# aelefebv/nellie

Measured on AMD Instinct MI355X. Metric: Mvoxel/s multiscale Frangi (5 sigma) + Label, float32, frame resident in HBM, higher is better.
Workload: dtype f32; 1 GPU; synthetic 1024x1024x1024 float32 volume (N(100,5) noise + Gaussian tube segments, seed 2345), 0.1 um isotropic, 5-scale Frangi + Label, full hot path per step, frame resident in HBM; voxels=1073741824, labels=265, one_pass_scales=5, fast_div_proven=2, hessian_tile_rows=16

## Files before the change

nellie_amd/csrc/hessian.inc:

```
struct VessP {
    float gamma_sq, alpha_sq, beta_sq;
    int use_thr;
    float thr;
    float max_abs, max_finite;
    int have_prev;
    int cnt_lo, cnt_hi;
    int first;
    float fsq_min;
    int m_inf;
    unsigned int *nan_flag;
    int all_ones;
    float fsq_lo, fsq_hi;
    int qcap;
    int zchunk;
    i64 idx_lo, idx_hi;
};

#define HM_TRACE_C 0.30f
#define HM_ENT 28
struct __attribute__((packed, aligned(4))) QEnt4 { float a, b, c, d; };
struct __attribute__((packed, aligned(4))) QEnt3 { float a, b, c; };
__device__ __forceinline__ void qent_store(float4 *region, unsigned int slot, float h0, float h1, float h2, float h3, float h4, float h5, unsigned int idx) {
    char *e = reinterpret_cast<char *>(region) + (size_t)__umul24(slot, (unsigned int)HM_ENT);
    *reinterpret_cast<QEnt4 *>(e) = QEnt4{h0, h1, h2, h3};
// ... 328 lines not shown
        mabs = wave_max_f(mabs); mfrob = wave_max_f(mfrob); anyinf = wave_or_i(anyinf);
        if ((tid & 63) == 0) { s_red[w] = mabs; s_red[16 + w] = mfrob; s_red[32 + w] = anyinf ? 1.0f : 0.0f; }
        __syncthreads();
        if (tid == 0) {
            float a = 0.0f, b = 0.0f, c = 0.0f;
            for (int k = 0; k < NT / 64; ++k) { a = fmaxf(a, s_red[k]); b = fmaxf(b, s_red[16 + k]); c = fmaxf(c, s_red[32 + k]); }
            if (a > 0.0f && __float_as_uint(a) > __hip_atomic_load(&res[0], __ATOMIC_RELAXED, __HIP_MEMORY_SCOPE_AGENT)) atomicMax(&res[0], __float_as_uint(a));
            if (b > 0.0f && __float_as_uint(b) > __hip_atomic_load(&res[1], __ATOMIC_RELAXED, __HIP_MEMORY_SCOPE_AGENT)) atomicMax(&res[1], __float_as_uint(b));
            if (c > 0.0f) atomicOr(&res[2], 1u);
        }
    }
    if (MODE != 0) {
        __syncthreads();
        if (lane == 0) {
            vq.count[region] = qn;
            if (MODE == 2 && qn > (unsigned int)vp.qcap) atomicOr(&res[3], 1u);
        }
        unsigned int *s_cnt = (unsigned int *)s_red;
        if (lane == 0) s_cnt[w] = cnt;
        __syncthreads();
        if (tid == 0) {
            unsigned long long t = 0;
            for (int k = 0; k < NT / 64; ++k) t += s_cnt[k];
            if (t) atomicAdd(mask_count, t);
        }
    }
}

template <bool RESOLVE>
__global__ void __launch_bounds__(256)
vesselness_queue_kernel(const float4 *__restrict__ ent, const unsigned int *__restrict__ count, unsigned int nregions,
                        float *__restrict__ vmax, i64 base, VessP vp, unsigned long long *cmask64,
                        const unsigned long long *pmask64, int wpr, int ny, int nx, i64 zbase,
                        unsigned long long *__restrict__ mask_count, const float *__restrict__ dev_params) {
    if (dev_params) { vp.gamma_sq = dev_params[2]; vp.fsq_min = dev_params[3]; vp.m_inf = __float_as_int(dev_params[4]); }
    unsigned int passed = 0;
    bool st_pending = false;
    i64 st_at = 0;
    float st_val = 0.0f;
    const unsigned int rstep = gridDim.x * 4u;
    unsigned int r = blockIdx.x * 4u + (threadIdx.x >> 6);
    unsigned int n_next = r < nregions ? count[r] : 0u;
    for (; r < nregions; r += rstep) {
    unsigned int n = n_next;
    n_next = (r + rstep < nregions) ? count[r + rstep] : 0u;
    if (RESOLVE && n > (unsigned int)vp.qcap) n = (unsigned int)vp.qcap;
    const float4 *e = ent + (size_t)r * (size_t)vp.qcap * 2;
    unsigned int i = threadIdx.x & 63u;
    float4 a = make_float4(0.f, 0.f, 0.f, 0.f), b = a;
    if (i < n) qent_load(e, i, a, b);
    asm volatile("" :: "v"(a.x), "v"(b.x));
    for (; i < n; i += 64u) {
        if (st_pending) { vmax[st_at] = st_val; st_pending = false; }
        const float4 a0 = a, b0 = b;
        if (i + 64u < n) qent_load(e, i + 64u, a, b);
        const float h[6] = {a0.x, a0.y, a0.z, a0.w, b0.x, b0.y};
        if (vp.all_ones) {
            if ((h[0] != h[0]) | (h[1] != h[1]) | (h[2] != h[2]) | (h[3] != h[3]) | (h[4] != h[4]) | (h[5] != h[5])) *vp.nan_flag = 1u;
        }
        unsigned int idx = __float_as_uint(b0.z);
        const bool undecided = RESOLVE && (idx & HM_UNDECIDED);
        idx &= ~HM_UNDECIDED;
        const i64 c = base + idx;
        const float cur = vp.first ? 0.0f : vmax[c];
        if (undecided) {
            const float fsq = frob_sq_of(h);
            if (!((fsq >= vp.fsq_min) && (fsq < __int_as_float(0x7f800000) || vp.m_inf))) continue;
            if ((i64)idx >= vp.idx_lo && (i64)idx < vp.idx_hi) ++passed;
            const i64 plane = (i64)ny * nx;
            const i64 zl = idx / plane;
            const int rem = (int)(idx - zl * plane);
            const int yy = rem / nx, xx = rem - yy * nx;
            const i64 word = ((zbase + zl) * ny + yy) * wpr + (xx >> 6);
            const unsigned long long bit = 1ull << (xx & 63);
            if (vp.have_prev && !(pmask64[word] & bit)) continue;
            atomicOr(&cmask64[word], bit);
            const float tr = h[0] + h[3] + h[5];
            if (!HM_TRACE_OK(tr, fsq)) continue;
        }
        float l1, l2, l3;
        eig3_sorted_abs(h, l1, l2, l3);
        const float val = frangi3(l1, l2, l3, vp.alpha_sq, vp.beta_sq, vp.gamma_sq);
        if (val > cur) { st_pending = true; st_at = c; st_val = val; }
    }
    }
    if (st_pending) vmax[st_at] = st_val;
    if (RESOLVE) {
        unsigned long long t = wave_sum_u64((unsigned long long)passed);
// ... 294 lines not shown
```

nellie_amd/csrc/label_runs.inc:

```

struct RunRec { int row; unsigned int x; };
struct RunN { const unsigned int *p; i64 h; i64 cap; };
__device__ __forceinline__ i64 run_n(const RunN &r) { const i64 n = r.p ? (i64)*r.p : r.h; return n > r.cap ? 0 : n; }

__device__ __forceinline__ unsigned long long rl_word(const unsigned long long *__restrict__ bits, i64 row, int w, int wpr,
                                                      int nx, bool invert) {
    unsigned long long v = bits[row * wpr + w];
    if (invert) v = ~v;
    const int rem = nx - w * 64;
    if (rem < 64) v &= (rem <= 0) ? 0ull : ((1ull << rem) - 1ull);
    return v;
}

__global__ void __launch_bounds__(256)
rl_threshold_pack_kernel(const float *__restrict__ f, const unsigned long long *__restrict__ support, unsigned long long *__restrict__ bits,
                         int has_thr, float thr_host, int nx, i64 nrows, int wpr, const float *__restrict__ thr_dev = nullptr) {
    const float thr = thr_dev ? *thr_dev : thr_host;
    const i64 wstride = ((i64)gridDim.x * blockDim.x) >> 6;
    const int lane = threadIdx.x & 63;
    const bool row_words = support && wpr <= 64;
    const i64 first = ((i64)blockIdx.x * blockDim.x + threadIdx.x) >> 6;
    unsigned long long mine_next = (row_words && first < nrows && lane < wpr) ? support[first * wpr + lane] : 0ull;
    unsigned long long st_res = 0ull;
    i64 st_row = -1;
// ... 430 lines not shown
    __syncthreads();
    const i64 base = chunk * RL_CHUNK;
    for (int k = threadIdx.x; k < RL_CHUNK; k += 256) {
        const i64 i = base + k;
        if (i >= nruns) break;
        const int root = parent[i];
        const int len = (int)(runs[i].x >> 16) - (int)(runs[i].x & 0xffffu);
        unsigned int h = ((unsigned int)root * 2654435761u) >> 24;
        bool done = false;
        for (int probe = 0; probe < 8 && !done; ++probe) {
            const int old = atomicCAS(&keys[h], -1, root);
            if (old == -1 || old == root) { atomicAdd(&vals[h], len); done = true; }
            else h = (h + 1) & (RL_HT - 1);
        }
        if (!done) atomicAdd(&area[root], len);
    }
    __syncthreads();
    for (int k = threadIdx.x; k < RL_HT; k += 256)
        if (keys[k] >= 0 && vals[k]) atomicAdd(&area[keys[k]], vals[k]);
  }
}

__global__ void __launch_bounds__(256)
rl_keep_kernel(const RunRec *__restrict__ runs, const int *__restrict__ parent, const int *__restrict__ area, int min_area,
               unsigned long long *__restrict__ bits, RunN rn, int wpr) {
    const i64 nruns = run_n(rn);
    for (i64 i = (i64)blockIdx.x * blockDim.x + threadIdx.x; i < nruns; i += (i64)gridDim.x * blockDim.x) {
        if (area[parent[i]] < min_area) continue;
        const RunRec r = runs[i];
        rl_set_bits(bits, r.row, wpr, (int)(r.x & 0xffffu), (int)(r.x >> 16));
    }
}

__global__ void __launch_bounds__(256)
majority_bits_kernel(const unsigned long long *__restrict__ in, unsigned long long *__restrict__ out, VolGeom v, int wpr, i64 z_lo, i64 z_hi) {
    const unsigned int ny = (unsigned int)v.ny, uw = (unsigned int)wpr;
    const unsigned int nw = (unsigned int)(z_hi - z_lo) * ny * uw;
    const unsigned int t0 = blockIdx.x * blockDim.x + threadIdx.x;
    if (t0 >= nw) return;
    const unsigned int w = t0 % uw, row0 = t0 / uw;
    const int y = (int)(row0 % ny), z = (int)(row0 / ny) + (int)z_lo;
    const i64 t = ((i64)z * ny + y) * wpr + w;
    const bool last = (w == uw - 1u);
    const unsigned long long top = 1ull << (((int)v.nx - 1) & 63);
    const unsigned long long valid = (top << 1) - 1ull;
    unsigned long long c0 = 0, c1 = 0, c2 = 0, c3 = 0, c4 = 0;
    auto add = [&](unsigned long long b) {
        unsigned long long t0_ = c0 & b; c0 ^= b; b = t0_;
        t0_ = c1 & b; c1 ^= b; b = t0_;
        t0_ = c2 & b; c2 ^= b; b = t0_;
        t0_ = c3 & b; c3 ^= b; b = t0_;
        c4 ^= b;
    };
    unsigned long long cw[9];
    i64 rws[9];
    unsigned long long any = 0ull;
#pragma unroll
    for (int dz = -1; dz <= 1; ++dz) {
        int zz = z + dz;
        const i64 gg = v.gz0 + zz;
        if (gg < 0 || gg >= v.gnz) zz = z;
#pragma unroll
        for (int dy = -1; dy <= 1; ++dy) {
            int yy = y + dy;
            yy = yy < 0 ? 0 : (yy >= (int)ny ? (int)ny - 1 : yy);
            const int k = (dz + 1) * 3 + (dy + 1);
            rws[k] = ((i64)zz * ny + yy) * wpr;
            cw[k] = in[rws[k] + w];
            any |= cw[k];
        }
    }
    if (any == 0ull) { out[t] = 0ull; return; }
#pragma unroll
    for (int k = 0; k < 9; ++k) {
        const unsigned long long cur = cw[k];
        const unsigned long long prev = (w > 0u) ? in[rws[k] + w - 1] : 0ull;
        const unsigned long long left = (cur << 1) | ((w > 0u) ? (prev >> 63) : (cur & 1ull));
        const unsigned long long next = last ? 0ull : in[rws[k] + w + 1];
        const unsigned long long right = (cur >> 1) | (last ? (cur & top) : (next << 63));
        add(left); add(cur); add(right);
    }
    unsigned long long res = c4 | (c3 & c2 & c1);
    if (last) res &= valid;
    out[t] = res;
}

__global__ void __launch_bounds__(256)
rl_paint_kernel(const unsigned long long *__restrict__ bits, const unsigned int *__restrict__ row_off, const int *__restrict__ parent,
                const int *__restrict__ newid, int *__restrict__ out, i64 row0, i64 row1, int wpr, int nx) {
    const i64 wstride = ((i64)gridDim.x * blockDim.x) >> 6;
    const int lane = threadIdx.x & 63;
    for (i64 row = row0 + (((i64)blockIdx.x * blockDim.x + threadIdx.x) >> 6); row < row1; row += wstride) {
        const unsigned int seen0 = row_off[row], nr = row_off[row + 1] - seen0;
        unsigned int seen = seen0;
        int *orow = out + (row - row0) * nx;
        const bool vec = ((nx & 3) == 0) && ((reinterpret_cast<size_t>(orow) & 15) == 0);
        if (nr == 0u && vec) {
            for (int q = lane; q < nx / 4; q += 64) reinterpret_cast<int4 *>(orow)[q] = make_int4(0, 0, 0, 0);
            continue;
        }
        const int lab_mine = ((unsigned int)lane < nr) ? newid[parent[seen0 + lane]] : 0;
        if (vec) {
            for (int q = lane; q < nx / 4; q += 64) reinterpret_cast<int4 *>(orow)[q] = make_int4(0, 0, 0, 0);
            asm volatile("s_waitcnt vmcnt(0)" ::: "memory");
            unsigned long long carry = 0;
            int prev_w = -2;
            for (int wb = 0; wb < wpr; wb += 64) {
                const unsigned long long mine = (wb + lane < wpr) ? rl_word(bits, row, wb + lane, wpr, nx, false) : 0ull;
                unsigned long long todo = __ballot(mine != 0ull);
                while (todo) {
                    const int wl = __builtin_ctzll(todo);
                    todo &= todo - 1;
                    const int w = wb + wl;
                    const unsigned long long v = __shfl(mine, wl, 64);
                    if (w != prev_w + 1) carry = 0ull;
                    const unsigned long long starts = v & ~((v << 1) | carry);
                    const int x = w * 64 + lane;
// ... 174 lines not shown
```

nellie_amd/csrc/nellie_hip.hip:

```cpp
#include "nl_host.h"

struct RcclApi {
    void *handle = nullptr;
    decltype(&ncclGetUniqueId) GetUniqueId = nullptr;
    decltype(&ncclCommInitRank) CommInitRank = nullptr;
    decltype(&ncclCommDestroy) CommDestroy = nullptr;
    decltype(&ncclGetErrorString) GetErrorString = nullptr;
    decltype(&ncclGroupStart) GroupStart = nullptr;
    decltype(&ncclGroupEnd) GroupEnd = nullptr;
    decltype(&ncclSend) Send = nullptr;
    decltype(&ncclRecv) Recv = nullptr;
    decltype(&ncclAllReduce) AllReduce = nullptr;
    decltype(&ncclBroadcast) Broadcast = nullptr;
    decltype(&ncclAllGather) AllGather = nullptr;
    bool ok = false;
};
static RcclApi &rccl_real() {
    static RcclApi api;
    if (!api.handle) {
        std::string rp;
        if (const char *e = getenv("ROCM_PATH")) rp = std::string(e) + "/lib/librccl.so.1";
        const char *names[] = {rp.c_str(), "/opt/rocm/lib/librccl.so.1", "/opt/rocm/lib/librccl.so", "librccl.so.1", "librccl.so"};
        for (const char *n : names) { if (!*n) continue; api.handle = dlopen(n, RTLD_NOW | RTLD_GLOBAL); if (api.handle) break; }
        if (api.handle) {
// ... 65 lines not shown
    return rccl_real().Broadcast(src, dst, count, dt, root, comm, st);
}
CommApi &rccl() { static CommApi api; return api; }

#include "sampling.inc"
#include "hessian.inc"
#include "hessian_pair.inc"
#include "hv_launch.h"
#include "filter2d.inc"
#include "thresholds.inc"
#include "chain.inc"
#include "percentile.inc"

static bool chain_unfused_sampling() {
    static int v = -1;
    if (v < 0) { const char *e = getenv("NELLIE_CHAIN_UNFUSED_SAMPLING"); v = (e && e[0] == '1') ? 1 : 0; }
    return v == 1;
}
static i64 sample_grid_cap() {
    static i64 v = 0;
    if (!v) { const char *e = getenv("NELLIE_SAMPLE_GRID"); v = (e && atoll(e) > 0) ? atoll(e) : 256; }
    return v;
}

bool gyx_tiled() {
    static int on = -1;
    if (on < 0) { const char *e = getenv("NELLIE_GYX_TILE"); on = (e && !atoi(e)) ? 0 : 1; }
    return on != 0;
}
static unsigned resolve_grid(unsigned blocks) {
    static long cap = -1;
    if (cap < 0) { const char *e = getenv("NELLIE_RESOLVE_GRID"); cap = e ? atol(e) : 8192; }
    return (cap > 0 && (unsigned)cap < blocks) ? (unsigned)cap : blocks;
}
static int hm_ty() {
    static int v = -1;
    if (v < 0) { const char *e = getenv("NELLIE_HM_TY"); v = (e && atoi(e) == 16) ? 16 : 8; }
    return v;
}
static int hv_rs_env() {
    static int v = -1;
    if (v < 0) { const char *e = getenv("NELLIE_HV_RS"); v = e ? atoi(e) : 8; if (v != 0 && v != 8 && !(NL_HV_VARIANTS && v == 16)) v = 8; }
    return v;
}
static int hv_rs(const nl_ctx *c) { return ((i64)(HM_ZCHUNK + 4) * c->ny * c->nx * 4 < ((i64)1 << 32)) ? hv_rs_env() : 0; }
static HessP hessp(const nl_ctx *c);
static HessDv<1> hessdv_fast(const nl_ctx *c) { return hessdv_fast(hessp(c)); }
static HessDv<0> hessdv_exact(const nl_ctx *c) { return hessdv_exact(hessp(c)); }
static int hv_fastv(const nl_ctx *c) { return c->fast_div2 ? 2 : (c->fast_div ? 1 : 0); }
static int hv_np(const nl_ctx *c) {
#if NL_HV_VARIANTS
    const char *e = getenv("NELLIE_HV_NP");
    return (e && atoi(e) == 2 && hv_rs(c) == 8 && hv_fastv(c) == 2) ? 2 : 1;
#else
    (void)c;
    return 1;
#endif
}
#define HD_SR 4
#define HD_COLS 60
static bool hv_dpp(const nl_ctx *c) {
    const char *e = getenv("NELLIE_HV_DPP");
    return hv_rs(c) != 0 && e && atoi(e) == 1;
}
static int hd_zchunk(const nl_ctx *c, i64 nz, i64 strips) {
    static int forced = -1;
// ... 1099 lines not shown
    NL_HIP(hipStreamSynchronize(st));
    *mask_count = (int64_t)(*h_cnt + c->spec_count);
    return NL_OK;
}

static bool resolve_on_side() {
    static int overlap = -1;
    if (overlap < 0) { const char *e = getenv("NELLIE_RESOLVE_OVERLAP"); overlap = (e && atoi(e)) ? 1 : 0; }
    return overlap != 0;
}
static int resolve_enqueue(nl_ctx *c, VessP vp, unsigned long long *d_cnt, const float *dev_params, char *err, size_t errlen, bool force_side = false) {
    const i64 plane = c->ny * c->nx, z0 = c->spec_z0, z1 = c->spec_z1;
    const bool side = force_side || resolve_on_side();
    hipStream_t st = side ? c->side : c->stream;
    if (side) {
        NL_HIP(hipEventRecord(c->ev_main, c->stream));
        NL_HIP(hipStreamWaitEvent(c->side, c->ev_main, 0));
    }
    vp.qcap = c->spec_qcap;
    vp.idx_lo = (c->own_lo - z0) * plane; vp.idx_hi = (c->own_hi - z0) * plane;
    {
        ProfScope ps(c, "vesselness_resolve", st);
        const int wpr = (int)((c->nx + 63) / 64);
        const i64 slot_words = c->nzl * c->ny * wpr;
        const int k_scale = c->mask_slots_used++;
        vp.have_prev = k_scale > 0;
        unsigned long long *cm = (unsigned long long *)c->m[0] + (i64)(k_scale & 1) * slot_words;
        const unsigned long long *pm = (unsigned long long *)c->m[0] + (i64)((k_scale + 1) & 1) * slot_words;
        if (vp.first && !vmax_is_zero(c, z0, z1))
            NL_HIP(hipMemsetAsync(c->f[c->i_vmax] + z0 * plane, 0, (size_t)(z1 - z0) * plane * 4, st));
        c->vmax_zero_hi = 0;
        vesselness_queue_kernel<true><<<resolve_grid((c->spec_nregions + 3) / 4), 256, 0, st>>>(
            (const float4 *)c->d_vq, c->d_vq_count, c->spec_nregions, c->f[c->i_vmax], z0 * plane, vp, cm, pm, wpr, (int)c->ny, (int)c->nx, z0, d_cnt,
            dev_params);
        NL_CHECK_LAUNCH();
    }
    if (side) {
        NL_HIP(hipEventRecord(c->ev_side, c->side));
        c->side_pending = 1;
    }
    c->spec_valid = 0;
    return NL_OK;
}

static bool resolve_defer_ok(const nl_ctx *c) {
    const char *e = getenv("NELLIE_RESOLVE_DEFER");
    const int on = e ? atoi(e) : 1;
    if (on == 2) return !c->comm && !resolve_on_side();
    return on && !c->comm && !c->ahead_pending && !resolve_on_side() && c->n >= ((i64)1 << 26);
}
static int resolve_deferred_launch(nl_ctx *c, bool on_side, char *err, size_t errlen) {
    if (!c->def_resolve) return NL_OK;
    c->def_resolve = 0;
    NL_JOIN_SIDE(c);
    VessP vp;
    static_assert(sizeof(VessP) <= sizeof(((nl_ctx *)nullptr)->def_vp), "nl_ctx::def_vp holds a VessP");
    memcpy(&vp, c->def_vp, sizeof(VessP));
    return resolve_enqueue(c, vp, c->def_cnt, c->def_params, err, errlen, on_side);
}

extern "C" int nl_vesselness_resolve(nl_ctx *c, float gamma_sq, float alpha_sq, float beta_sq, int use_thr, float thr,
                                     int *hit, int64_t *mask_count, char *err, size_t errlen) {
    NL_ENTER(c);
    if (!hit) return nl_fail(err, errlen, NL_EINVAL, "hit is NULL");
    *hit = 0;
    if (!c->spec_valid) return NL_OK;
    VessP vp = make_vessp(c, gamma_sq, alpha_sq, beta_sq, use_thr, thr);
// ... 272 lines not shown
    } else {
        ProfScope ps(c, "vesselness");
        const int ntx = (int)((c->nx + HM_TX - 1) / HM_TX);
        const int wpr = (int)((c->nx + 63) / 64);
        const i64 slot_words = c->nzl * c->ny * wpr;
        const int k_scale = c->mask_slots_used++;
        vp.have_prev = k_scale > 0;
        unsigned long long *cm = (unsigned long long *)c->m[0] + (i64)(k_scale & 1) * slot_words;
        const unsigned long long *pm = (unsigned long long *)c->m[0] + (i64)((k_scale + 1) & 1) * slot_words;
        const i64 plane = c->ny * c->nx;
        const i64 planes_per_launch = (i64)c->vq_chunks * HM_ZCHUNK;
        const VQueue vq{(float4 *)c->d_vq, c->d_vq_count};
        if (vp.first && !vmax_is_zero(c, z0, z1))
            NL_HIP(hipMemsetAsync(c->f[c->i_vmax] + z0 * plane, 0, (size_t)(z1 - z0) * plane * 4, c->stream));
        c->vmax_zero_hi = 0;
        const int rs = hv_rs(c);
        const int ty = rs ? 2 * rs : hm_ty();
        const int nty = (int)((c->ny + ty - 1) / ty);
        if (rs) vp.qcap = 2 * hv_np(c) * HM_REGION;
#define NL_LAUNCH_VESS(TYV, FASTV, HR)                                                                                    \
        hessian_g_kernel<1, TYV, FASTV><<<nblocks, HGCfg<TYV>::NT, HGCfg<TYV>::lds_bytes(), c->stream>>>(                 \
            gauss_cur(c), cm, pm, wpr, geom(c), HR, vp, vq, (int)za, (int)zb, ntx, nty, nullptr, d_cnt)
        for (i64 za = z0; za < z1; za += planes_per_launch) {
            const i64 zb = za + planes_per_launch < z1 ? za + planes_per_launch : z1;
            const int nzc = (int)((zb - za + HM_ZCHUNK - 1) / HM_ZCHUNK);
            const unsigned nblocks = (unsigned)(ntx * nty * nzc);
            if (rs) NL_HIP(nl_hv_launch(HvLaunch{1, rs, hv_np(c), hv_fastv(c), nblocks, c->stream, gauss_cur(c), cm, pm, wpr, geom(c), hessp(c), vp, vq, (int)za, (int)zb,
                                                 ntx, nty, nullptr, d_cnt, nullptr}));
            else if (ty == 8) { if (c->fast_div) NL_LAUNCH_VESS(8, true, hessdv_fast(c)); else NL_LAUNCH_VESS(8, false, hessdv_exact(c)); }
            else { if (c->fast_div) NL_LAUNCH_VESS(16, true, hessdv_fast(c)); else NL_LAUNCH_VESS(16, false, hessdv_exact(c)); }
            NL_CHECK_LAUNCH();
            const unsigned nregions = nblocks * (unsigned)(rs ? rs / hv_np(c) : ty);
            vesselness_queue_kernel<false><<<resolve_grid((nregions + 3) / 4), 256, 0, c->stream>>>(vq.ent, vq.count, nregions, c->f[c->i_vmax], za * plane, vp,
                                                                                      nullptr, nullptr, wpr, (int)c->ny, (int)c->nx, za, nullptr, nullptr);
            NL_CHECK_LAUNCH();
        }
#undef NL_LAUNCH_VESS
        NL_CHECK_LAUNCH();
    }
    if (mask_count) {
        NL_HIP(hipMemcpyAsync(c->h_small, d_cnt, 8, hipMemcpyDeviceToHost, c->stream));
        NL_HIP(hipStreamSynchronize(c->stream));
        *mask_count = (int64_t)(*(unsigned long long *)c->h_small);
    }
    return NL_OK;
}

extern "C" int nl_set_ndim(nl_ctx *c, int ndim, char *err, size_t errlen) {
    NL_ENTER(c);
    if (ndim != 2 && ndim != 3) return nl_fail(err, errlen, NL_EINVAL, "ndim must be 2 or 3");
    if (ndim == 2 && (c->nzl != 1 || c->gnz != 1)) return nl_fail(err, errlen, NL_EINVAL, "a 2-D context has exactly one plane");
    c->two_d = ndim == 2;
    c->fsq_cache_valid = 0;
    return NL_OK;
}

extern "C" int nl_log2d_step(nl_ctx *c, const double *wy2, const double *wy0, const double *wx2, const double *wx0, int r,
                             float s2, int first, int use_mask, char *err, size_t errlen) {
    NL_ENTER(c);
    if (!c->two_d) return nl_fail(err, errlen, NL_ESTATE, "nl_log2d_step on a 3-D context");
    if (!wy2 || !wy0 || !wx2 || !wx0) return nl_fail(err, errlen, NL_EINVAL, "weights are NULL");
    NL_JOIN_SIDE(c);
    for (int k = 0; k < 4; ++k)
        if (!c->d_2d[k]) NL_HIP(hipMalloc((void **)&c->d_2d[k], (size_t)c->n * 4));
    GaussW gy2, gy0, gx2, gx0;
    int rc;
    if ((rc = fill_gw(gy2, wy2, r, err, errlen)) || (rc = fill_gw(gy0, wy0, r, err, errlen)) ||
// ... 696 lines not shown
    NL_HIP(zero_small(d_n, 4, c->stream));
    {
        ProfScope ps(c, "sample");
        flat_gather_pos_kernel<<<(unsigned)((count + 255) / 256), 256, 0, c->stream>>>(src, -c->gz0 * plane, offset + k0 * step, step, count, stage, d_n);
        NL_CHECK_LAUNCH();
    }
    return fetch_counted(c, stage, d_n, count, out, cap, n, err, errlen);
}


extern "C" int nl_ctx_info(nl_ctx *c, const char *key, double *value) {
    if (!c || !key || !value) return NL_EINVAL;
    if (!strcmp(key, "fast_div")) *value = c->fast_div2 ? 2 : c->fast_div;
    else if (!strcmp(key, "hessian_tile_rows")) *value = hv_rs(c) ? 2 * hv_rs(c) : hm_ty();
    else if (!strcmp(key, "hv_variants")) *value = NL_HV_VARIANTS;
    else if (!strcmp(key, "vesselness_one_pass")) *value = c->spec_ok;
    else if (!strcmp(key, "chain_available")) *value = (c->two_d || (c->spec_ok && hv_rs(c))) ? 1 : 0;
    else if (!strcmp(key, "last_fsq_min")) *value = c->last_fsq_min;
    else if (!strcmp(key, "last_spec_overflow")) *value = c->last_spec_overflow;
    else if (!strcmp(key, "last_label_sparse")) *value = c->last_label_sparse;
    else if (!strcmp(key, "device_bytes")) *value = (double)nl_ctx_bytes(c->nzl, c->ny, c->nx);
    else if (!strcmp(key, "gauss_yx_max_r")) *value = getenv("NELLIE_NO_FUSED_YX") ? 0 : GM_MAX_R;
    else if (!strcmp(key, "queue_entries")) {
        if (hipSetDevice(c->device) != hipSuccess) return NL_EHIP;
        if (c->side_pending && hipStreamSynchronize(c->side) != hipSuccess) return NL_EHIP;
        const unsigned nreg = c->spec_nregions;
        std::vector<unsigned int> h(nreg);
        if (nreg && (hipMemcpyAsync(h.data(), c->d_vq_count, (size_t)nreg * 4, hipMemcpyDeviceToHost, c->stream) != hipSuccess ||
                     hipStreamSynchronize(c->stream) != hipSuccess)) return NL_EHIP;
        double t = 0.0;
        for (unsigned k = 0; k < nreg; ++k) t += (double)h[k];
        *value = t;
    }
    else if (!strcmp(key, "nan_hessian")) {
        if (hipSetDevice(c->device) != hipSuccess) return NL_EHIP;
        unsigned int flag = 0;
        if (c->side_pending && hipStreamSynchronize(c->side) != hipSuccess) return NL_EHIP;
        if (hipMemcpyAsync(&flag, (char *)c->d_small + NL_NAN_FLAG_OFF, 4, hipMemcpyDeviceToHost, c->stream) != hipSuccess ||
            hipStreamSynchronize(c->stream) != hipSuccess) return NL_EHIP;
        *value = flag ? 1.0 : 0.0;
    }
    else return NL_EINVAL;
    return NL_OK;
}

extern "C" int nl_debug_eig_frangi(nl_ctx *c, const float *h6, int64_t n, int impl, float alpha_sq, float beta_sq,
                                   float gamma_sq, float *out4, char *err, size_t errlen) {
    NL_ENTER(c);
    if (!h6 || !out4 || n < 1 || n * 6 > c->n) return nl_fail(err, errlen, NL_EINVAL, "bad debug batch (n=%lld)", (i64)n);
    float *d_in = c->f[(c->i_gauss + 1) % 3], *d_out = c->f[(c->i_gauss + 2) % 3];
    NL_HIP(hipMemcpyAsync(d_in, h6, (size_t)n * 24, hipMemcpyHostToDevice, c->stream));
    debug_eig_kernel<<<(unsigned)((n + 255) / 256), 256, 0, c->stream>>>(d_in, n, impl, alpha_sq, beta_sq, gamma_sq, d_out);
    NL_CHECK_LAUNCH();
    NL_HIP(hipMemcpyAsync(out4, d_out, (size_t)n * 16, hipMemcpyDeviceToHost, c->stream));
    NL_HIP(hipStreamSynchronize(c->stream));
    return NL_OK;
}

extern "C" int nl_timer_begin(nl_ctx *c, char *err, size_t errlen) {
    NL_ENTER(c);
    NL_HIP(hipEventRecord(c->t0, c->stream));
    return NL_OK;
}
extern "C" int nl_timer_end_ms(nl_ctx *c, float *ms, char *err, size_t errlen) {
    NL_ENTER(c);
    NL_HIP(hipEventRecord(c->t1, c->stream));
// ... 47 lines not shown
```

nellie_amd/csrc/nellie_label.hip:

```cpp
#include "nl_host.h"
#include "label_voxels.inc"
#include "label_runs.inc"
#include "pack_out.inc"
#include "network.inc"

extern "C" int nl_label_load_frangi(nl_ctx *c, const float *host, int64_t z0, int64_t z1, char *err, size_t errlen) {
    NL_ENTER(c);
    if (!host || z0 < 0 || z1 > c->nzl || z0 >= z1) return nl_fail(err, errlen, NL_EINVAL, "bad plane range [%lld,%lld)", (i64)z0, (i64)z1);
    const i64 plane = c->ny * c->nx;
    c->i_vmax = 3; c->i_gauss = 0; c->i_labels = -1;
    NL_HIP(hipMemcpyAsync(c->f[c->i_vmax] + z0 * plane, host, (size_t)(z1 - z0) * plane * 4, hipMemcpyHostToDevice, c->stream));
    NL_HIP(hipStreamSynchronize(c->stream));
    c->frangi_ready = 1;
    return NL_OK;
}

extern "C" int nl_label_intensity_mask_planes(nl_ctx *c, const void *host_original, int dtype, double thresh, int64_t z0, int64_t z1,
                                              char *err, size_t errlen) {
    NL_ENTER(c);
    if (z0 < 0 || z1 > c->nzl || z0 >= z1) return nl_fail(err, errlen, NL_EINVAL, "bad plane range [%lld,%lld)", (i64)z0, (i64)z1);
    const i64 count = (z1 - z0) * c->ny * c->nx;
    const size_t es = dtype_size(dtype);
    if (!es || !host_original) return nl_fail(err, errlen, NL_EINVAL, "bad original image (dtype code %d)", dtype);
    void *raw = nullptr;
// ... 260 lines not shown
    uint8_t *flag = c->m[0];
    const VolGeom vg{g.nz, g.ny, g.nx, g.gz0, g.gnz};
    int rc;
    *overflow = false;
    static int dev_count = -1;
    if (dev_count < 0) { const char *e = getenv("NELLIE_LABEL_HOST_COUNTS"); dev_count = (e && atoi(e)) ? 0 : 1; }
    rs.host_count = !dev_count;
    NL_HIP(zero_small((unsigned int *)c->d_small + 60, 4, c->stream));
    auto known_empty = [&]() { return rs.host_count && rs.nruns == 0; };
    if (fill_holes) {
        if ((rc = build_components<6>(c, g, g.bitsA, 1, rs, cap, overflow, err, errlen))) return rc;
        if (*overflow) return NL_OK;
        if (!known_empty()) {
            const unsigned gr = run_blocks(rs, g.nrows);
            rl_fill_u8_kernel<<<gr, 256, 0, c->stream>>>(flag, rs.rn());
            rl_border_kernel<<<gr, 256, 0, c->stream>>>(rs.runs, rs.parent, flag, rs.rn(), vg);
            NL_CHECK_LAUNCH();
            rl_fill_kernel<<<gr, 256, 0, c->stream>>>(rs.runs, rs.parent, flag, g.bitsA, rs.rn(), g.wpr);
            NL_CHECK_LAUNCH();
        }
    }
    if ((rc = build_components<26>(c, g, g.bitsA, 0, rs, cap, overflow, err, errlen))) return rc;
    if (*overflow) return NL_OK;
    NL_HIP(hipMemsetAsync(g.bitsB, 0, (size_t)g.nwords * 8, c->stream));
    if (!known_empty()) {
        const unsigned gr = run_blocks(rs, g.nrows);
        rl_fill_u32_kernel<<<gr, 256, 0, c->stream>>>((unsigned int *)aux, 0u, rs.rn());
        rl_area_kernel<<<run_blocks(rs, g.nrows / 16 + 1, RL_CHUNK), 256, 0, c->stream>>>(rs.runs, rs.parent, aux, rs.rn());
        NL_CHECK_LAUNCH();
        const int ma = (int)(min_area > 0x7fffffff ? 0x7fffffff : min_area);
        rl_keep_kernel<<<gr, 256, 0, c->stream>>>(rs.runs, rs.parent, aux, ma, g.bitsB, rs.rn(), g.wpr);
        NL_CHECK_LAUNCH();
    }
    majority_bits_kernel<<<(unsigned)((g.nwords + 255) / 256), 256, 0, c->stream>>>(g.bitsB, g.bitsA, vg, g.wpr, 0, g.nz);
    NL_CHECK_LAUNCH();
    if ((rc = build_components<26>(c, g, g.bitsA, 0, rs, cap, overflow, err, errlen))) return rc;
    if (*overflow) return NL_OK;
    if ((rc = number_and_paint(c, g, rs, aux, n_labels, err, errlen, overflow))) return rc;
    if (*overflow) return NL_OK;
    c->i_labels = free_idx[2];
    return NL_OK;
}

static int label_out_index(const nl_ctx *c) {
    int last = -1;
    for (int k = 0; k < 4; ++k) if (k != c->i_vmax) last = k;
    return last;
}

extern "C" int nl_label_run(nl_ctx *c, int has_thr, float thr, int64_t min_area, int fill_holes, int64_t *n_labels,
                            char *err, size_t errlen) {
    NL_ENTER(c);
    if (!c->frangi_ready) return nl_fail(err, errlen, NL_ESTATE, "nl_label_run before a Frangi volume exists");
    if (c->nzl != c->gnz) return nl_fail(err, errlen, NL_EINVAL, "nl_label_run works on a whole volume (Z-slabs: nl_label_pack / nl_label_run_global)");
    static int force_voxel = -1;
    if (force_voxel < 0) { const char *e = getenv("NELLIE_LABEL_VOXEL"); force_voxel = (e && atoi(e)) ? 1 : 0; }
    if (force_voxel || c->nx > 65535) return label_run_voxels(c, has_thr, thr, min_area, fill_holes, n_labels, err, errlen);
    LabelGeo g;
    g.nz = c->nzl; g.ny = c->ny; g.nx = c->nx;
    g.nrows = c->nzl * c->ny; g.wpr = (int)((c->nx + 63) / 64); g.nwords = g.nrows * g.wpr;
    g.rows = c->d_rows;
    g.bitsA = (unsigned long long *)c->m[1]; g.bitsB = (unsigned long long *)c->m[2];
    g.paint_row0 = 0; g.paint_row1 = g.nrows; g.paint_out = (int *)c->f[label_out_index(c)];
    g.link_scratch = g.paint_out;
    label_geo_whole(g);
    g.whole_frame_paint = true;
    c->pack_pending = 0;
// ... 295 lines not shown
    if ((rc = slab_host_stage(c, (size_t)2 * n, err, errlen))) return rc;
    memcpy(c->h_sl, roots, (size_t)n * 4); memcpy(c->h_sl + n, values, (size_t)n * 4);
    int *d_idx = sg.stage, *d_val = sg.stage + n;
    NL_HIP(hipMemcpyAsync(d_idx, c->h_sl, (size_t)2 * n * 4, hipMemcpyHostToDevice, c->stream));
    sl_patch_kernel<<<(unsigned)((n + 255) / 256), 256, 0, c->stream>>>(sg.aux, c->sl_phase == SL_FILL ? c->m[0] : nullptr, d_idx, d_val, (int)n);
    NL_CHECK_LAUNCH();
    return NL_OK;
}

extern "C" int nl_slab_apply(nl_ctx *c, int64_t min_area, char *err, size_t errlen) {
    NL_ENTER(c);
    if (c->sl_phase != SL_FILL && c->sl_phase != SL_AREA) return nl_fail(err, errlen, NL_ESTATE, "nl_slab_apply outside the fill / area phases");
    SlabGeo sg; int rc = slab_geo(c, sg, err, errlen); if (rc) return rc;
    LabelGeo &g = sg.g; RunSet &rs = sg.rs;
    ProfScope ps(c, "label");
    const unsigned gr = (unsigned)((rs.nruns + 255) / 256);
    if (c->sl_phase == SL_FILL) {
        if (rs.nruns) sl_fill_kernel<<<gr, 256, 0, c->stream>>>(rs.runs, rs.parent, c->m[0], g.bitsA, rs.nruns, g.wpr, sg.row_lo, sg.row_hi);
    } else {
        NL_HIP(hipMemsetAsync(g.bitsB + (i64)sg.row_lo * g.wpr, 0, (size_t)(sg.row_hi - sg.row_lo) * g.wpr * 8, c->stream));
        const int ma = (int)(min_area > 0x7fffffff ? 0x7fffffff : min_area);
        if (rs.nruns) sl_keep_kernel<<<gr, 256, 0, c->stream>>>(rs.runs, rs.parent, sg.aux, ma, g.bitsB, rs.nruns, g.wpr, sg.row_lo, sg.row_hi);
    }
    NL_CHECK_LAUNCH();
    return NL_OK;
}

extern "C" int nl_slab_majority(nl_ctx *c, char *err, size_t errlen) {
    NL_ENTER(c);
    SlabGeo sg; int rc = slab_geo(c, sg, err, errlen); if (rc) return rc;
    LabelGeo &g = sg.g;
    ProfScope ps(c, "label");
    const i64 z_lo = c->own_lo - c->sl_e0, z_hi = c->own_hi - c->sl_e0;
    majority_bits_kernel<<<(unsigned)(((z_hi - z_lo) * g.ny * g.wpr + 255) / 256), 256, 0, c->stream>>>(g.bitsB, g.bitsA, VolGeom{g.nz, g.ny, g.nx, g.gz0, g.gnz}, g.wpr, z_lo, z_hi);
    NL_CHECK_LAUNCH();
    return NL_OK;
}

extern "C" int nl_slab_number(nl_ctx *c, int64_t n_clear, const int32_t *clear, int64_t n_set, const int32_t *set, int64_t *n_local,
                              int32_t *ids_of_set, char *err, size_t errlen) {
    NL_ENTER(c);
    if (c->sl_phase != SL_NUMBER) return nl_fail(err, errlen, NL_ESTATE, "nl_slab_number outside the numbering phase");
    if (n_clear < 0 || n_set < 0 || (n_clear && !clear) || (n_set && (!set || !ids_of_set)) || n_clear + n_set > c->n / 4) return nl_fail(err, errlen, NL_EINVAL, "bad selection lists");
    SlabGeo sg; int rc = slab_geo(c, sg, err, errlen); if (rc) return rc;
    RunSet &rs = sg.rs;
    ProfScope ps(c, "label");
    unsigned long long total = 0;
    if (rs.nruns) {
        sl_select_kernel<<<(unsigned)((rs.nruns + 255) / 256), 256, 0, c->stream>>>(rs.runs, rs.parent, sg.sel, rs.nruns, sg.row_lo, sg.row_hi);
        int *d_idx = (int *)(sg.scan + rs.nruns);
        if (rs.nruns + n_clear + 2 * n_set > sg.cap) return nl_fail(err, errlen, NL_ENOMEM, "selection lists do not fit the scratch volume [out of memory]");
        if ((rc = slab_host_stage(c, (size_t)(n_clear + n_set) + 2 + (size_t)n_set, err, errlen))) return rc;
        if (n_clear) memcpy(c->h_sl, clear, (size_t)n_clear * 4);
        if (n_set) memcpy(c->h_sl + n_clear, set, (size_t)n_set * 4);
        if (n_clear + n_set) NL_HIP(hipMemcpyAsync(d_idx, c->h_sl, (size_t)(n_clear + n_set) * 4, hipMemcpyHostToDevice, c->stream));
        if (n_clear) sl_set_u32_kernel<<<(unsigned)((n_clear + 255) / 256), 256, 0, c->stream>>>(sg.sel, d_idx, (int)n_clear, 0u);
        if (n_set) sl_set_u32_kernel<<<(unsigned)((n_set + 255) / 256), 256, 0, c->stream>>>(sg.sel, d_idx + n_clear, (int)n_set, 1u);
        NL_CHECK_LAUNCH();
        if ((rc = scan_excl_u32(c, sg.sel, sg.scan, rs.nruns, err, errlen))) return rc;
        int *h_back = c->h_sl + n_clear + n_set;
        int *d_out = d_idx + n_clear + n_set;
        if (n_set) {
            sl_gather_kernel<<<(unsigned)((n_set + 255) / 256), 256, 0, c->stream>>>(sg.scan, d_idx + n_clear, d_out, (int)n_set, 1);
            NL_CHECK_LAUNCH();
            NL_HIP(hipMemcpyAsync(h_back + 2, d_out, (size_t)n_set * 4, hipMemcpyDeviceToHost, c->stream));
        }
        NL_HIP(hipMemcpyAsync(h_back, sg.scan + rs.nruns - 1, 4, hipMemcpyDeviceToHost, c->stream));
// ... 470 lines not shown
```

Before: 28390 Mvoxel/s.

## Pack queue regions per wave and stream majority filter along z

The vesselness queue kernel now gives each wave a contiguous run of regions (or a strided run when NELLIE_RESOLVE_DEAL=1). It prefix-sums up to 16 region counts so that partially filled regions are packed into full 64-lane iterations instead of one region per wave pass. The 3x3x3 majority filter is restructured so that each wave walks a 16-plane z chunk. It reuses per-plane bit-sliced 9-neighbour counts across z with ripple adders, and gets word-edge bits from neighbouring lanes through shuffles instead of extra global loads. A diagnostic query for padded queue slots is also added. The changes add lane-locate overhead per entry and give fewer, longer-running waves in the majority kernel.

New measurement: 28620 Mvoxel/s (median of 6 runs). Within noise of the previous version (+0.8%).

```diff
diff --git a/nellie_amd/csrc/hessian.inc b/nellie_amd/csrc/hessian.inc
--- a/nellie_amd/csrc/hessian.inc
+++ b/nellie_amd/csrc/hessian.inc
@@ -384,28 +384,59 @@
 vesselness_queue_kernel(const float4 *__restrict__ ent, const unsigned int *__restrict__ count, unsigned int nregions,
                         float *__restrict__ vmax, i64 base, VessP vp, unsigned long long *cmask64,
                         const unsigned long long *pmask64, int wpr, int ny, int nx, i64 zbase,
-                        unsigned long long *__restrict__ mask_count, const float *__restrict__ dev_params) {
+                        unsigned long long *__restrict__ mask_count, const float *__restrict__ dev_params, int deal) {
     if (dev_params) { vp.gamma_sq = dev_params[2]; vp.fsq_min = dev_params[3]; vp.m_inf = __float_as_int(dev_params[4]); }
     unsigned int passed = 0;
     bool st_pending = false;
     i64 st_at = 0;
     float st_val = 0.0f;
-    const unsigned int rstep = gridDim.x * 4u;
-    unsigned int r = blockIdx.x * 4u + (threadIdx.x >> 6);
-    unsigned int n_next = r < nregions ? count[r] : 0u;
-    for (; r < nregions; r += rstep) {
-    unsigned int n = n_next;
-    n_next = (r + rstep < nregions) ? count[r + rstep] : 0u;
-    if (RESOLVE && n > (unsigned int)vp.qcap) n = (unsigned int)vp.qcap;
-    const float4 *e = ent + (size_t)r * (size_t)vp.qcap * 2;
-    unsigned int i = threadIdx.x & 63u;
+    const unsigned int lane = threadIdx.x & 63u;
+    const unsigned int nwaves = gridDim.x * 4u;
+    const unsigned int wid = (unsigned int)__builtin_amdgcn_readfirstlane((int)(blockIdx.x * 4u + (threadIdx.x >> 6)));
+    unsigned int rfirst, rstride, nmine;
+    if (deal == 0) {
+        const unsigned int per = (nregions + nwaves - 1u) / nwaves;
+        rfirst = wid * per; rstride = 1u;
+        nmine = rfirst < nregions ? (nregions - rfirst < per ? nregions - rfirst : per) : 0u;
+    } else {
+        rfirst = wid; rstride = nwaves;
+        nmine = wid < nregions ? (nregions - wid + nwaves - 1u) / nwaves : 0u;
+    }
+    unsigned int n_next = (lane < 16u && lane < nmine) ? count[rfirst + lane * rstride] : 0u;
+    for (unsigned int bat = 0; bat < nmine; bat += 16u) {
+    unsigned int ends = n_next;
+    n_next = (lane < 16u && bat + 16u + lane < nmine) ? count[rfirst + (bat + 16u + lane) * rstride] : 0u;
+    if (RESOLVE && ends > (unsigned int)vp.qcap) ends = (unsigned int)vp.qcap;
+#pragma unroll
+    for (int d = 1; d < 16; d <<= 1) {
+        const unsigned int up = (unsigned int)__shfl_up((int)ends, d, 64);
+        if (lane >= (unsigned int)d) ends += up;
+    }
+    const unsigned int nb = nmine - bat < 16u ? nmine - bat : 16u;
+    const unsigned int n = (unsigned int)__builtin_amdgcn_readlane((int)ends, (int)(nb - 1u));
+    const float4 *const ebase = ent + (size_t)(rfirst + bat * rstride) * (size_t)vp.qcap * 2;
+    const size_t estride = (size_t)rstride * (size_t)vp.qcap * 2;
+    auto locate = [&](const unsigned int g, const float4 *&e, unsigned int &slot) {
+        unsigned int k = 0u, start = 0u;
+        for (unsigned int j = 0; j + 1u < nb; ++j) {
+            const unsigned int ej = (unsigned int)__builtin_amdgcn_readlane((int)ends, (int)j);
+            if (g >= ej) { k = j + 1u; start = ej; }
+        }
+        e = ebase + (size_t)k * estride;
+        slot = g - start;
+    };
+    unsigned int i = lane;
     float4 a = make_float4(0.f, 0.f, 0.f, 0.f), b = a;
-    if (i < n) qent_load(e, i, a, b);
+    const float4 *e;
+    unsigned int slot;
+    locate(i, e, slot);
+    if (i < n) qent_load(e, slot, a, b);
     asm volatile("" :: "v"(a.x), "v"(b.x));
     for (; i < n; i += 64u) {
         if (st_pending) { vmax[st_at] = st_val; st_pending = false; }
         const float4 a0 = a, b0 = b;
-        if (i + 64u < n) qent_load(e, i + 64u, a, b);
+        locate(i + 64u, e, slot);
+        if (i + 64u < n) qent_load(e, slot, a, b);
         const float h[6] = {a0.x, a0.y, a0.z, a0.w, b0.x, b0.y};
         if (vp.all_ones) {
             if ((h[0] != h[0]) | (h[1] != h[1]) | (h[2] != h[2]) | (h[3] != h[3]) | (h[4] != h[4]) | (h[5] != h[5])) *vp.nan_flag = 1u;
diff --git a/nellie_amd/csrc/label_runs.inc b/nellie_amd/csrc/label_runs.inc
--- a/nellie_amd/csrc/label_runs.inc
+++ b/nellie_amd/csrc/label_runs.inc
@@ -486,57 +486,99 @@
     }
 }
 
+#define MAJ_ZC 16
+struct MajP { unsigned long long c0, c1, c2, c3, any; };
+__device__ __forceinline__ void maj_add1(MajP &p, unsigned long long b) {
+    unsigned long long t = p.c0 & b; p.c0 ^= b; b = t;
+    t = p.c1 & b; p.c1 ^= b; b = t;
+    t = p.c2 & b; p.c2 ^= b; b = t;
+    p.c3 ^= b;
+}
 __global__ void __launch_bounds__(256)
 majority_bits_kernel(const unsigned long long *__restrict__ in, unsigned long long *__restrict__ out, VolGeom v, int wpr, i64 z_lo, i64 z_hi) {
     const unsigned int ny = (unsigned int)v.ny, uw = (unsigned int)wpr;
-    const unsigned int nw = (unsigned int)(z_hi - z_lo) * ny * uw;
-    const unsigned int t0 = blockIdx.x * blockDim.x + threadIdx.x;
-    if (t0 >= nw) return;
-    const unsigned int w = t0 % uw, row0 = t0 / uw;
-    const int y = (int)(row0 % ny), z = (int)(row0 / ny) + (int)z_lo;
-    const i64 t = ((i64)z * ny + y) * wpr + w;
+    const unsigned int pw = ny * uw;
+    const unsigned int nstrips = (pw + 63u) / 64u;
+    const unsigned int lane = threadIdx.x & 63u;
+    const unsigned int wave = (unsigned int)__builtin_amdgcn_readfirstlane((int)(blockIdx.x * 4u + (threadIdx.x >> 6)));
+    const unsigned int chunk = wave / nstrips;
+    const i64 zc0 = z_lo + (i64)chunk * MAJ_ZC;
+    if (zc0 >= z_hi) return;
+    const i64 zc1 = zc0 + MAJ_ZC < z_hi ? zc0 + MAJ_ZC : z_hi;
+    const unsigned int p = (wave - chunk * nstrips) * 64u + lane;
+    const bool ok = p < pw;
+    const unsigned int w = p % uw, y = p / uw;
+    const unsigned int pm = (y > 0u ? y - 1u : 0u) * uw + w, pp = (y + 1u < ny ? y + 1u : ny - 1u) * uw + w;
     const bool last = (w == uw - 1u);
     const unsigned long long top = 1ull << (((int)v.nx - 1) & 63);
     const unsigned long long valid = (top << 1) - 1ull;
-    unsigned long long c0 = 0, c1 = 0, c2 = 0, c3 = 0, c4 = 0;
-    auto add = [&](unsigned long long b) {
-        unsigned long long t0_ = c0 & b; c0 ^= b; b = t0_;
-        t0_ = c1 & b; c1 ^= b; b = t0_;
-        t0_ = c2 & b; c2 ^= b; b = t0_;
-        t0_ = c3 & b; c3 ^= b; b = t0_;
-        c4 ^= b;
-    };
-    unsigned long long cw[9];
-    i64 rws[9];
-    unsigned long long any = 0ull;
+    const bool edge_lo = ok && lane == 0u && w > 0u, edge_hi = ok && lane == 63u && !last;
+    const int eoff = edge_lo ? -1 : 1;
+
+    struct Raw { unsigned long long r0, r1, r2, e0, e1, e2; };
+    auto load = [&](const i64 z) {
+        const unsigned long long *pl = in + z * (i64)pw;
+        Raw r{0ull, 0ull, 0ull, 0ull, 0ull, 0ull};
+        if (ok) { r.r0 = pl[pm]; r.r1 = pl[p]; r.r2 = pl[pp]; }
+        if (edge_lo || edge_hi) { r.e0 = pl[(int)pm + eoff]; r.e1 = pl[(int)p + eoff]; r.e2 = pl[(int)pp + eoff]; }
+        return r;
+    };
+    auto count9 = [&](const Raw &r) {
+        MajP P{0ull, 0ull, 0ull, 0ull, r.r0 | r.r1 | r.r2 | r.e0 | r.e1 | r.e2};
+        if (__ballot(P.any != 0ull) == 0ull) return P;
+        const unsigned int sb = (unsigned int)(r.r0 >> 63) | ((unsigned int)(r.r1 >> 63) << 1) | ((unsigned int)(r.r2 >> 63) << 2) |
+                                ((unsigned int)(r.r0 & 1ull) << 3) | ((unsigned int)(r.r1 & 1ull) << 4) | ((unsigned int)(r.r2 & 1ull) << 5);
+        unsigned int from_lo = (unsigned int)__shfl_up((int)sb, 1, 64), from_hi = (unsigned int)__shfl_down((int)sb, 1, 64) >> 3;
+        if (lane == 0u) from_lo = (unsigned int)(r.e0 >> 63) | ((unsigned int)(r.e1 >> 63) << 1) | ((unsigned int)(r.e2 >> 63) << 2);
+        if (lane == 63u) from_hi = (unsigned int)(r.e0 & 1ull) | ((unsigned int)(r.e1 & 1ull) << 1) | ((unsigned int)(r.e2 & 1ull) << 2);
+        const unsigned long long cw[3] = {r.r0, r.r1, r.r2};
 #pragma unroll
-    for (int dz = -1; dz <= 1; ++dz) {
-        int zz = z + dz;
-        const i64 gg = v.gz0 + zz;
-        if (gg < 0 || gg >= v.gnz) zz = z;
-#pragma unroll
-        for (int dy = -1; dy <= 1; ++dy) {
-            int yy = y + dy;
-            yy = yy < 0 ? 0 : (yy >= (int)ny ? (int)ny - 1 : yy);
-            const int k = (dz + 1) * 3 + (dy + 1);
-            rws[k] = ((i64)zz * ny + yy) * wpr;
-            cw[k] = in[rws[k] + w];
-            any |= cw[k];
-        }
-    }
-    if (any == 0ull) { out[t] = 0ull; return; }
-#pragma unroll
-    for (int k = 0; k < 9; ++k) {
-        const unsigned long long cur = cw[k];
-        const unsigned long long prev = (w > 0u) ? in[rws[k] + w - 1] : 0ull;
-        const unsigned long long left = (cur << 1) | ((w > 0u) ? (prev >> 63) : (cur & 1ull));
-        const unsigned long long next = last ? 0ull : in[rws[k] + w + 1];
-        const unsigned long long right = (cur >> 1) | (last ? (cur & top) : (next << 63));
-        add(left); add(cur); add(right);
-    }
-    unsigned long long res = c4 | (c3 & c2 & c1);
-    if (last) res &= valid;
-    out[t] = res;
+        for (int k = 0; k < 3; ++k) {
+            const unsigned long long cur = cw[k];
+            const unsigned long long left = (cur << 1) | ((w > 0u) ? (unsigned long long)((from_lo >> k) & 1u) : (cur & 1ull));
+            const unsigned long long right = (cur >> 1) | (last ? (cur & top) : ((unsigned long long)((from_hi >> k) & 1u) << 63));
+            maj_add1(P, left); maj_add1(P, cur); maj_add1(P, right);
+        }
+        return P;
+    };
+    auto fa = [](unsigned long long a, unsigned long long b, unsigned long long &cy) {
+        const unsigned long long x = a ^ b, s = x ^ cy;
+        cy = (a & b) | (cy & x);
+        return s;
+    };
+
+    const bool has_lo = v.gz0 + zc0 - 1 >= 0;
+    Raw nxt = load(zc0);
+    Raw rlo = has_lo ? load(zc0 - 1) : nxt;
+    MajP Pc = count9(nxt);
+    MajP Pm = has_lo ? count9(rlo) : Pc;
+    bool has_next = v.gz0 + zc0 + 1 < v.gnz;
+    if (has_next) nxt = load(zc0 + 1);
+    for (i64 z = zc0; z < zc1; ++z) {
+        const Raw cur = nxt;
+        const bool has_next2 = z + 1 < zc1 && v.gz0 + z + 2 < v.gnz;
+        if (has_next2) nxt = load(z + 2);
+        const MajP Pp = has_next ? count9(cur) : Pc;
+        unsigned long long res = 0ull;
+        if (__ballot((Pm.any | Pc.any | Pp.any) != 0ull) != 0ull) {
+            unsigned long long cy = 0ull;
+            const unsigned long long s0 = fa(Pm.c0, Pc.c0, cy), s1 = fa(Pm.c1, Pc.c1, cy), s2 = fa(Pm.c2, Pc.c2, cy), s3 = fa(Pm.c3, Pc.c3, cy);
+            const unsigned long long s4 = cy;
+            cy = 0ull;
+            (void)fa(s0, Pp.c0, cy);
+            const unsigned long long t1 = fa(s1, Pp.c1, cy), t2 = fa(s2, Pp.c2, cy), t3 = fa(s3, Pp.c3, cy);
+            const unsigned long long t4 = s4 ^ cy;
+            res = t4 | (t3 & t2 & t1);
+            if (last) res &= valid;
+        }
+        if (ok) out[z * (i64)pw + p] = res;
+        Pm = Pc; Pc = Pp;
+        has_next = has_next2;
+    }
+}
+static inline unsigned majority_blocks(i64 planes, i64 ny, int wpr) {
+    const i64 strips = (ny * wpr + 63) / 64, chunks = (planes + MAJ_ZC - 1) / MAJ_ZC;
+    return (unsigned)((strips * chunks + 3) / 4);
 }
 
 __global__ void __launch_bounds__(256)
diff --git a/nellie_amd/csrc/nellie_hip.hip b/nellie_amd/csrc/nellie_hip.hip
--- a/nellie_amd/csrc/nellie_hip.hip
+++ b/nellie_amd/csrc/nellie_hip.hip
@@ -121,6 +121,11 @@
     static long cap = -1;
     if (cap < 0) { const char *e = getenv("NELLIE_RESOLVE_GRID"); cap = e ? atol(e) : 8192; }
     return (cap > 0 && (unsigned)cap < blocks) ? (unsigned)cap : blocks;
+}
+static int resolve_deal() {
+    static int v = -1;
+    if (v < 0) { const char *e = getenv("NELLIE_RESOLVE_DEAL"); v = (e && atoi(e) == 1) ? 1 : 0; }
+    return v;
 }
 static int hm_ty() {
     static int v = -1;
@@ -1286,7 +1291,7 @@
         c->vmax_zero_hi = 0;
         vesselness_queue_kernel<true><<<resolve_grid((c->spec_nregions + 3) / 4), 256, 0, st>>>(
             (const float4 *)c->d_vq, c->d_vq_count, c->spec_nregions, c->f[c->i_vmax], z0 * plane, vp, cm, pm, wpr, (int)c->ny, (int)c->nx, z0, d_cnt,
-            dev_params);
+            dev_params, resolve_deal());
         NL_CHECK_LAUNCH();
     }
     if (side) {
@@ -1625,7 +1630,7 @@
             NL_CHECK_LAUNCH();
             const unsigned nregions = nblocks * (unsigned)(rs ? rs / hv_np(c) : ty);
             vesselness_queue_kernel<false><<<resolve_grid((nregions + 3) / 4), 256, 0, c->stream>>>(vq.ent, vq.count, nregions, c->f[c->i_vmax], za * plane, vp,
-                                                                                      nullptr, nullptr, wpr, (int)c->ny, (int)c->nx, za, nullptr, nullptr);
+                                                                                      nullptr, nullptr, wpr, (int)c->ny, (int)c->nx, za, nullptr, nullptr, resolve_deal());
             NL_CHECK_LAUNCH();
         }
 #undef NL_LAUNCH_VESS
@@ -2388,6 +2393,17 @@
         for (unsigned k = 0; k < nreg; ++k) t += (double)h[k];
         *value = t;
     }
+    else if (!strcmp(key, "queue_region_slots")) {
+        if (hipSetDevice(c->device) != hipSuccess) return NL_EHIP;
+        if (c->side_pending && hipStreamSynchronize(c->side) != hipSuccess) return NL_EHIP;
+        const unsigned nreg = c->spec_nregions;
+        std::vector<unsigned int> h(nreg);
+        if (nreg && (hipMemcpyAsync(h.data(), c->d_vq_count, (size_t)nreg * 4, hipMemcpyDeviceToHost, c->stream) != hipSuccess ||
+                     hipStreamSynchronize(c->stream) != hipSuccess)) return NL_EHIP;
+        double t = 0.0;
+        for (unsigned k = 0; k < nreg; ++k) t += (double)(((h[k] + 63u) / 64u) * 64u);
+        *value = t;
+    }
     else if (!strcmp(key, "nan_hessian")) {
         if (hipSetDevice(c->device) != hipSuccess) return NL_EHIP;
         unsigned int flag = 0;
diff --git a/nellie_amd/csrc/nellie_label.hip b/nellie_amd/csrc/nellie_label.hip
--- a/nellie_amd/csrc/nellie_label.hip
+++ b/nellie_amd/csrc/nellie_label.hip
@@ -316,7 +316,7 @@
         rl_keep_kernel<<<gr, 256, 0, c->stream>>>(rs.runs, rs.parent, aux, ma, g.bitsB, rs.rn(), g.wpr);
         NL_CHECK_LAUNCH();
     }
-    majority_bits_kernel<<<(unsigned)((g.nwords + 255) / 256), 256, 0, c->stream>>>(g.bitsB, g.bitsA, vg, g.wpr, 0, g.nz);
+    majority_bits_kernel<<<majority_blocks(g.nz, g.ny, g.wpr), 256, 0, c->stream>>>(g.bitsB, g.bitsA, vg, g.wpr, 0, g.nz);
     NL_CHECK_LAUNCH();
     if ((rc = build_components<26>(c, g, g.bitsA, 0, rs, cap, overflow, err, errlen))) return rc;
     if (*overflow) return NL_OK;
@@ -678,7 +678,7 @@
     LabelGeo &g = sg.g;
     ProfScope ps(c, "label");
     const i64 z_lo = c->own_lo - c->sl_e0, z_hi = c->own_hi - c->sl_e0;
-    majority_bits_kernel<<<(unsigned)(((z_hi - z_lo) * g.ny * g.wpr + 255) / 256), 256, 0, c->stream>>>(g.bitsB, g.bitsA, VolGeom{g.nz, g.ny, g.nx, g.gz0, g.gnz}, g.wpr, z_lo, z_hi);
+    majority_bits_kernel<<<majority_blocks(z_hi - z_lo, g.ny, g.wpr), 256, 0, c->stream>>>(g.bitsB, g.bitsA, VolGeom{g.nz, g.ny, g.nx, g.gz0, g.gnz}, g.wpr, z_lo, z_hi);
     NL_CHECK_LAUNCH();
     return NL_OK;
 }
```
